# arpitbansal297/Cold-Diffusion-Models

Measured on NVIDIA H100. Metric: training-step images/sec (CelebA-128 deblur UNet, config 3), higher is better.
Workload: dtype tf32

## Files before the change

### cold_diffusion_models_b200/csrc/wgrad_tc.cu

```cuda
#include "tc_common.cuh"

namespace {

constexpr int kMmaWarps = 8;
constexpr int kThreads = 32 * (kMmaWarps + 1);
constexpr int kMaxTaps = 8;
constexpr int kMaxGroups = 4;
constexpr int kMaxAccCols = 256;

struct WgParams {
  int B, Hg, Wg;
  int CW, R, KR;
  int chunks_x, chunks_y, total_chunks, chunks_per_split, splits;
  int Cout, Cin;
  int tiles_co, tiles_ci;
  int ngroups;
  int ntaps[kMaxGroups];
  int nloads[kMaxGroups];
  int tap_index[kMaxGroups][kMaxTaps];
  int tap_load[kMaxGroups][kMaxTaps];
  int tap_shift[kMaxGroups][kMaxTaps];
  int load_dy[kMaxGroups][kMaxTaps], load_dx[kMaxGroups][kMaxTaps];
  int halo;
  int sy, sx;
  int oys, oxs, oy0, ox0;
  int per_batch, chunks_per_img, splits_per_img;
  long long dw_batch_stride;
  float* dw;
  float* db;
  int wm_nbox[kMaxGroups], ci_tile;
  int wm_box[kMaxGroups][kMaxTaps][2], wm_shift[kMaxGroups][kMaxTaps][2], wm_tap[kMaxGroups][kMaxTaps][2];
};

__device__ __forceinline__ float lds_sw(const uint8_t* base, int row, int c) {
  return cd_round_tf32(*reinterpret_cast<const float*>(base + row * 128 + ((((c >> 2) ^ row) & 7) << 4) + (c & 3) * 4));
}
__device__ __forceinline__ void mma_tf32_16x8x8(float (&d)[4], const float (&a)[4], const float (&b)[2]) {
  asm volatile("mma.sync.aligned.m16n8k8.row.col.f32.tf32.tf32.f32 {%0, %1, %2, %3}, {%4, %5, %6, %7}, {%8, %9}, {%0, %1, %2, %3};"
               : "+f"(d[0]), "+f"(d[1]), "+f"(d[2]), "+f"(d[3])
               : "r"(__float_as_uint(a[0])), "r"(__float_as_uint(a[1])), "r"(__float_as_uint(a[2])), "r"(__float_as_uint(a[3])),
                 "r"(__float_as_uint(b[0])), "r"(__float_as_uint(b[1])));
}
__device__ __forceinline__ void red_add_v2(float* addr, float a, float b) {
  asm volatile("red.global.add.v2.f32 [%0], {%1, %2};" :: "l"(addr), "f"(a), "f"(b) : "memory");
}

template <int BN, int NT, bool BIAS>
__global__ void __launch_bounds__(kThreads, 1)
wgrad_tc_kernel(const __grid_constant__ CUtensorMap mapDY, const __grid_constant__ CUtensorMap mapX,
                const WgParams p, int stages, int a_bytes, int b_bytes, int b_tx_bytes) {
  constexpr int NCH = BN / 32;
  constexpr int NJ = BN / 16;
  static_assert(NT * BN <= kMaxAccCols, "accumulators of one CTA");
  extern __shared__ uint8_t smem_raw[];
  const uint32_t raw_addr = smem_u32(smem_raw);
  uint8_t* smem = smem_raw + ((1024u - (raw_addr & 1023u)) & 1023u);
  const int g = blockIdx.z;
  const int nl = p.nloads[g];
  const int stage_bytes = a_bytes + nl * b_bytes;
  uint64_t* bars = reinterpret_cast<uint64_t*>(smem + stages * stage_bytes);
  uint64_t* full_bar = bars;
  uint64_t* empty_bar = bars + stages;
  const int warp = threadIdx.x >> 5, lane = threadIdx.x & 31;

  if (threadIdx.x == 0) {
    for (int i = 0; i < stages; ++i) { mbar_init(&full_bar[i], 1); mbar_init(&empty_bar[i], kMmaWarps); }
    asm volatile("fence.mbarrier_init.release.cluster;" ::: "memory");
  }
  __syncthreads();

  const int tile = blockIdx.x;
  const int co0 = (tile % p.tiles_co) * 128, ci0 = (tile / p.tiles_co) * BN;
  const int split = blockIdx.y;
  int c_beg = split * p.chunks_per_split;
  int c_end = c_beg + p.chunks_per_split; if (c_end > p.total_chunks) c_end = p.total_chunks;
  long long dw_off = 0;
  if (p.per_batch) {
    const int n = split / p.splits_per_img, sp = split % p.splits_per_img;
    c_beg = n * p.chunks_per_img + sp * p.chunks_per_split;
    c_end = c_beg + p.chunks_per_split;
    if (c_end > (n + 1) * p.chunks_per_img) c_end = (n + 1) * p.chunks_per_img;
    dw_off = n * p.dw_batch_stride;
  }
  const int nchunks = c_end > c_beg ? c_end - c_beg : 0;

  if (warp == kMmaWarps) {
    for (int it = 0; it < nchunks; ++it) {
      const int c = c_beg + it;
      const int cx = c % p.chunks_x;
      const int cy = (c / p.chunks_x) % p.chunks_y;
      const int n = c / (p.chunks_x * p.chunks_y);
      const int gx0 = cx * p.CW, gy0 = cy * p.R;
      const uint32_t stage = it % stages, ph = (it / stages) & 1u;
      mbar_wait(&empty_bar[stage], ph ^ 1u);
      if (elect_one()) {
        mbar_expect_tx(&full_bar[stage], a_bytes + nl * b_tx_bytes);
        const uint32_t sa = smem_u32(smem + stage * stage_bytes);
#pragma unroll
        for (int ch = 0; ch < 4; ++ch)
          tma_load_4d(sa + ch * (a_bytes / 4), &mapDY, &full_bar[stage], co0 + ch * 32, gx0 * p.oxs + p.ox0, gy0 * p.oys + p.oy0, n);
        for (int l = 0; l < nl; ++l) {
          const uint32_t sb = sa + a_bytes + l * b_bytes;
          const int xin = gx0 * p.sx + p.load_dx[g][l], yin = gy0 * p.sy + p.load_dy[g][l];
          for (int ch = 0; ch < NCH; ++ch)
            tma_load_4d(sb + ch * (b_bytes / NCH), &mapX, &full_bar[stage], ci0 + ch * 32, xin, yin, n);
        }
      }
      __syncwarp();
    }
    return;
  }

  const int wm = warp & 3, wn = warp >> 2;
  const int gq = lane >> 2, tq = lane & 3;
  const bool bias_cta = BIAS && p.db != nullptr && (tile / p.tiles_co) == 0 && g == 0 && wn == 0;
  int tap_load[NT], tap_shift[NT];
#pragma unroll
  for (int t = 0; t < NT; ++t) { tap_load[t] = p.tap_load[g][t]; tap_shift[t] = p.tap_shift[g][t]; }
  float acc[NT][2][NJ][4];
#pragma unroll
  for (int t = 0; t < NT; ++t)
#pragma unroll
    for (int i = 0; i < 2; ++i)
#pragma unroll
      for (int j = 0; j < NJ; ++j)
#pragma unroll
        for (int e = 0; e < 4; ++e) acc[t][i][j][e] = 0.f;
  float bsum[2][2] = {{0.f, 0.f}, {0.f, 0.f}};
  const int ksteps = p.KR / 8, cw_shift = __ffs(p.CW) - 1, rowlen = p.CW + p.halo;
  for (int it = 0; it < nchunks; ++it) {
    const uint32_t stage = it % stages, ph = (it / stages) & 1u;
    mbar_wait(&full_bar[stage], ph);
    const uint8_t* sA = smem + stage * stage_bytes + wm * (a_bytes / 4);
    const uint8_t* sB = smem + stage * stage_bytes + a_bytes;
#pragma unroll 1
    for (int ks = 0; ks < ksteps; ++ks) {
      const int k0 = ks * 8 + tq, k1 = k0 + 4;
      float a[2][4];
#pragma unroll
      for (int i = 0; i < 2; ++i) {
        a[i][0] = lds_sw(sA, k0, i * 16 + gq);
        a[i][1] = lds_sw(sA, k0, i * 16 + gq + 8);
        a[i][2] = lds_sw(sA, k1, i * 16 + gq);
        a[i][3] = lds_sw(sA, k1, i * 16 + gq + 8);
        if (bias_cta) { bsum[i][0] += a[i][0] + a[i][2]; bsum[i][1] += a[i][1] + a[i][3]; }
      }
      const int r0 = (k0 >> cw_shift) * rowlen + (k0 & (p.CW - 1)), r1 = (k1 >> cw_shift) * rowlen + (k1 & (p.CW - 1));
#pragma unroll
      for (int t = 0; t < NT; ++t) {
        const uint8_t* sBt = sB + tap_load[t] * b_bytes;
#pragma unroll
        for (int j = 0; j < NJ; ++j) {
          const int cl = wn * (BN / 2) + j * 8 + gq;
          const uint8_t* sBc = sBt + (cl >> 5) * (b_bytes / NCH);
          const float b[2] = {lds_sw(sBc, r0 + tap_shift[t], cl & 31), lds_sw(sBc, r1 + tap_shift[t], cl & 31)};
          mma_tf32_16x8x8(acc[t][0][j], a[0], b);
          mma_tf32_16x8x8(acc[t][1][j], a[1], b);
        }
      }
    }
    __syncwarp();
    if (lane == 0) mbar_arrive(&empty_bar[stage]);
  }
  if (nchunks == 0) return;
#pragma unroll
  for (int t = 0; t < NT; ++t) {
    if (t >= p.ntaps[g]) break;
#pragma unroll
    for (int i = 0; i < 2; ++i) {
#pragma unroll
      for (int h = 0; h < 2; ++h) {
        const int co = co0 + wm * 32 + i * 16 + gq + h * 8;
        if (co >= p.Cout) continue;
        float* wrow = p.dw + dw_off + (static_cast<long long>(p.tap_index[g][t]) * p.Cout + co) * p.Cin;
#pragma unroll
        for (int j = 0; j < NJ; ++j) {
          const int ci = ci0 + wn * (BN / 2) + j * 8 + tq * 2;
          if (ci < p.Cin) red_add_v2(wrow + ci, acc[t][i][j][2 * h], acc[t][i][j][2 * h + 1]);
        }
      }
    }
  }
  if (BIAS && bias_cta) {
#pragma unroll
    for (int i = 0; i < 2; ++i)
#pragma unroll
      for (int h = 0; h < 2; ++h) {
        float v = bsum[i][h];
        v += __shfl_xor_sync(0xffffffffu, v, 1);
        v += __shfl_xor_sync(0xffffffffu, v, 2);
        const int co = co0 + wm * 32 + i * 16 + gq + h * 8;
        if (tq == 0 && co < p.Cout) atomicAdd(p.db + co, v);
      }
  }
}

constexpr int kWmThreads = 512;
constexpr int kWmKR = 64;
constexpr int kWmRegsLow = 40, kWmRegsHigh = 216;

template <int CW, bool HALO> struct WmGeom {
  static constexpr int R = kWmKR / CW, RL = HALO ? CW + 8 : CW;
  static constexpr int kXBox = RL * (R + (HALO ? 2 : 0)) * 128;
  static_assert(kXBox % 1024 == 0, "X boxes keep 1024-byte alignment");
};
template <int BN> struct WmTiles {
  static constexpr int kRawBox = kWmKR * 128;
  static constexpr int kRawBytes = (BN / 32) * kRawBox;
  static constexpr int kBBytes = BN * kWmKR * 4;
};
constexpr int wm_slots_1x1(int BN) { return BN == 128 ? 3 : 4; }
template <int BN, int CW, bool HALO> struct WmStage {
  static constexpr int kXBytes = (HALO ? 2 : 2 * wm_slots_1x1(BN)) * WmGeom<CW, HALO>::kXBox;
  static constexpr int kBytes = WmTiles<BN>::kRawBytes + WmTiles<BN>::kBBytes + kXBytes;
  static_assert((224 * 1024) / kBytes >= 2, "two stages of the wgmma weight-gradient kernel fit shared memory");
};

template <int BN, int NTW, int CW, bool HALO>
__device__ __forceinline__ void wm_consume(const WgParams& p, const uint8_t* smem, int stages, int stage_bytes,
                                           uint64_t* afull, uint64_t* aempty, uint64_t* bfull, uint64_t* bempty, int nchunks, int g,
                                           int tbeg, int co0, int ci0) {
  using G = WmGeom<CW, HALO>;
  using T = WmTiles<BN>;
  const int lane = threadIdx.x & 31, w = (threadIdx.x & 127) >> 5, gq = lane >> 2, tq = lane & 3;
  int off[NTW][2];
  const int c = 16 * (w & 1) + gq;
#pragma unroll
  for (int t = 0; t < NTW; ++t) {
#pragma unroll
    for (int h = 0; h < 2; ++h) {
      const int row = ((NTW <= 2 && p.Cin == 32) ? p.wm_shift[g][tbeg + t][w >> 1] : p.wm_shift[g][tbeg + t][0]) + 2 * tq + h;
      const int box = (NTW <= 2 && p.Cin == 32) ? 0 : (HALO ? 0 : 2 * (tbeg + t)) + (w >> 1);
      off[t][h] = box * G::kXBox + row * 128 + ((((c >> 2) ^ row) & 7) << 4) + (c & 3) * 4;
    }
  }
  float acc[NTW][BN / 2];
  uint32_t fr[2][NTW][4];
  auto load_frags = [&](uint32_t (&f)[NTW][4], const uint8_t* xs, int ks) {
    const int kofs = (((ks * 8) / CW) * G::RL + (ks * 8) % CW) * 128;
#pragma unroll
    for (int t = 0; t < NTW; ++t)
#pragma unroll
      for (int e = 0; e < 4; ++e)
        f[t][e] = __float_as_uint(cd_round_tf32(*reinterpret_cast<const float*>(xs + (off[t][e >> 1] ^ ((e & 1) * 32)) + kofs)));
  };
  if (nchunks == 0) return;
  mbar_wait(&afull[0], 0);
  load_frags(fr[0], smem + T::kRawBytes + T::kBBytes, 0);
  for (int it = 0; it < nchunks; ++it) {
    const uint32_t s = it % stages, ph = (it / stages) & 1u;
    mbar_wait(&bfull[s], ph);
    const uint8_t* xs = smem + s * stage_bytes + T::kRawBytes + T::kBBytes;
    const uint32_t bs = smem_u32(smem + s * stage_bytes + T::kRawBytes);
#pragma unroll
    for (int ks = 0; ks < kWmKR / 8; ++ks) {
      wgmma_fence();
      const uint64_t db = make_kmajor_sw128_desc(bs + (ks >> 2) * (BN * 128)) + uint64_t((ks & 3) * 2);
#pragma unroll
      for (int t = 0; t < NTW; ++t) wgmma_tf32_rs<BN>(acc[t], fr[ks & 1][t], db, (it | ks) != 0 ? 1u : 0u);
      wgmma_commit();
      if (ks + 1 < kWmKR / 8) {
        load_frags(fr[(ks + 1) & 1], xs, ks + 1);
      } else if (it + 1 < nchunks) {
        const uint32_t s1 = (it + 1) % stages, ph1 = ((it + 1) / stages) & 1u;
        mbar_wait(&afull[s1], ph1);
        load_frags(fr[0], smem + s1 * stage_bytes + T::kRawBytes + T::kBBytes, 0);
      }
      wgmma_wait<0>();
    }
    __syncwarp();
    if (lane == 0) { mbar_arrive(&aempty[s]); mbar_arrive(&bempty[s]); }
  }
  asm volatile("" ::: "memory");
  const long long dw_off = p.per_batch ? (blockIdx.y / p.splits_per_img) * p.dw_batch_stride : 0;
#pragma unroll
  for (int t = 0; t < NTW; ++t) {
    const int tap = p.wm_tap[g][tbeg + t][w >> 1];
    if (tap < 0) continue;
    float* wt = p.dw + dw_off + static_cast<long long>(tap) * p.Cout * p.Cin + ci0 + 32 * p.wm_box[g][tbeg + t][w >> 1] +
                16 * (w & 1) + gq;
#pragma unroll
    for (int j = 0; j < BN / 8; ++j)
#pragma unroll
      for (int e = 0; e < 4; ++e) {
        const int co = co0 + 8 * j + 2 * tq + (e & 1);
        if (co < p.Cout) atomicAdd(wt + static_cast<long long>(co) * p.Cin + (e >> 1) * 8, acc[t][4 * j + e]);
      }
  }
}

template <int BN, int NT, int CW, bool HALO>
__global__ void __launch_bounds__(kWmThreads, 1)
wgrad_wgmma_kernel(const __grid_constant__ CUtensorMap mapDY, const __grid_constant__ CUtensorMap mapX, const __grid_constant__ WgParams p,
                   int stages) {
  using G = WmGeom<CW, HALO>;
  using T = WmTiles<BN>;
  constexpr int kStage = WmStage<BN, CW, HALO>::kBytes;
  extern __shared__ uint8_t smem_raw[];
  const uint32_t raw_addr = smem_u32(smem_raw);
  uint8_t* smem = smem_raw + ((1024u - (raw_addr & 1023u)) & 1023u);
  uint64_t* bars = reinterpret_cast<uint64_t*>(smem + stages * kStage);
  uint64_t* afull = bars;
  uint64_t* aempty = bars + stages;
  uint64_t* rfull = bars + 2 * stages;
  uint64_t* rempty = bars + 3 * stages;
  uint64_t* bfull = bars + 4 * stages;
  uint64_t* bempty = bars + 5 * stages;
  const int warp = threadIdx.x >> 5, lane = threadIdx.x & 31, wg = threadIdx.x >> 7;
  const int g = blockIdx.z, nt = p.ntaps[g];
  const int ncons = nt > 1 ? 2 : 1;
  if (threadIdx.x == 0) {
    for (int i = 0; i < stages; ++i) {
      mbar_init(&afull[i], 1); mbar_init(&aempty[i], 4 * ncons);
      mbar_init(&rfull[i], 1); mbar_init(&rempty[i], 4);
      mbar_init(&bfull[i], 4); mbar_init(&bempty[i], 4 * ncons);
    }
    asm volatile("fence.mbarrier_init.release.cluster;" ::: "memory");
  }
  __syncthreads();

  const int tile = blockIdx.x;
  const int co0 = (tile % p.tiles_co) * BN, ci0 = (tile / p.tiles_co) * p.ci_tile;
  int c_beg = blockIdx.y * p.chunks_per_split;
  int c_end = c_beg + p.chunks_per_split; if (c_end > p.total_chunks) c_end = p.total_chunks;
  if (p.per_batch) {
    const int n = blockIdx.y / p.splits_per_img, sp = blockIdx.y % p.splits_per_img;
    c_beg = n * p.chunks_per_img + sp * p.chunks_per_split;
    c_end = c_beg + p.chunks_per_split;
    if (c_end > (n + 1) * p.chunks_per_img) c_end = (n + 1) * p.chunks_per_img;
  }
  const int nchunks = c_end > c_beg ? c_end - c_beg : 0;

  if (wg == 0) {
    asm volatile("setmaxnreg.dec.sync.aligned.u32 %0;" :: "n"(kWmRegsLow));
    if (warp != 0) return;
    for (int it = 0; it < nchunks; ++it) {
      const int ch = c_beg + it;
      const int gx0 = (ch % p.chunks_x) * CW, gy0 = ((ch / p.chunks_x) % p.chunks_y) * G::R, n = ch / (p.chunks_x * p.chunks_y);
      const uint32_t s = it % stages, ph = (it / stages) & 1u;
      const uint32_t sx = smem_u32(smem + s * kStage);
      mbar_wait(&rempty[s], ph ^ 1u);
      if (elect_one()) {
        mbar_expect_tx(&rfull[s], T::kRawBytes);
#pragma unroll
        for (int b = 0; b < BN / 32; ++b)
          tma_load_4d(sx + b * T::kRawBox, &mapDY, &rfull[s], co0 + 32 * b, gx0, gy0, n);
      }
      __syncwarp();
      mbar_wait(&aempty[s], ph ^ 1u);
      if (elect_one()) {
        const int nb = p.wm_nbox[g], h = HALO ? 1 : 0;
        mbar_expect_tx(&afull[s], nb * G::kXBox);
        for (int b = 0; b < nb; ++b)
          tma_load_4d(sx + T::kRawBytes + T::kBBytes + b * G::kXBox, &mapX, &afull[s], ci0 + 32 * b, gx0 - h, gy0 - h, n);
      }
      __syncwarp();
    }
    return;
  }
  if (wg == 1) {
    asm volatile("setmaxnreg.dec.sync.aligned.u32 %0;" :: "n"(kWmRegsLow));
    const int w4 = warp & 3;
    for (int it = 0; it < nchunks; ++it) {
      const uint32_t s = it % stages, ph = (it / stages) & 1u;
      mbar_wait(&rfull[s], ph);
      mbar_wait(&bempty[s], ph ^ 1u);
      const uint8_t* raw = smem + s * kStage;
      uint8_t* bt = smem + s * kStage + T::kRawBytes;
#pragma unroll 4
      for (int u = w4; u < (BN / 32) * (kWmKR / 4); u += 4) {
        const int b = u % (BN / 32), kq = u / (BN / 32);
        const int co = 32 * b + lane;
        const uint8_t* src = raw + b * T::kRawBox + (lane & 3) * 4;
        float v[4];
#pragma unroll
        for (int j = 0; j < 4; ++j) {
          const int px = 8 * (kq >> 1) + (kq & 1) + 2 * j;
          v[j] = cd_round_tf32(*reinterpret_cast<const float*>(src + px * 128 + ((((lane >> 2) ^ px) & 7) << 4)));
        }
        *reinterpret_cast<float4*>(bt + (kq >> 3) * (BN * 128) + co * 128 + (((kq ^ co) & 7) << 4)) = make_float4(v[0], v[1], v[2], v[3]);
      }
      asm volatile("fence.proxy.async.shared::cta;" ::: "memory");
      __syncwarp();
      if (lane == 0) { mbar_arrive(&rempty[s]); mbar_arrive(&bfull[s]); }
    }
    return;
  }
  const int half = (nt + 1) / 2;
  const int tbeg = (wg - 2) * half;
  const int ntw = wg == 2 ? half : nt - half;
  if (ntw <= 0) return;
  asm volatile("setmaxnreg.inc.sync.aligned.u32 %0;" :: "n"(kWmRegsHigh));
#define WM_CONSUME(n) wm_consume<BN, n, CW, HALO>(p, smem, stages, kStage, afull, aempty, bfull, bempty, nchunks, g, tbeg, co0, ci0)
  if constexpr (NT == 4 && HALO) {
    if (ntw == 4) WM_CONSUME(4);
    else if (ntw == 3) WM_CONSUME(3);
    else if (ntw == 2) WM_CONSUME(2);
    else WM_CONSUME(1);
  } else {
    if (ntw == 2) WM_CONSUME(2);
    else WM_CONSUME(1);
  }
#undef WM_CONSUME
}

int g_wg_mode = 1;

constexpr int kMaxSmem = 224 * 1024 + 1024 + 256;

template <int BN, int NT>
int launch_wg(bool bias, dim3 grid, size_t smem, cudaStream_t st, const CUtensorMap& mapDY, const CUtensorMap& mapX,
              const WgParams& p, int stages, int a_bytes, int b_bytes, int b_tx) {
  constexpr auto with_bias = wgrad_tc_kernel<BN, NT, true>, without = wgrad_tc_kernel<BN, NT, false>;
  CD_CUDA(bias ? smem_limit_once<with_bias>(kMaxSmem) : smem_limit_once<without>(kMaxSmem));
  auto kern = bias ? with_bias : without;
  kern<<<grid, kThreads, smem, st>>>(mapDY, mapX, p, stages, a_bytes, b_bytes, b_tx);
  CD_LAUNCH_CHECK();
  return 0;
}

}

extern "C" int cd_wgrad_tc_set_mode(int mode) { g_wg_mode = mode; return 0; }

static int g_wg_bias_fusion = 0;
extern "C" int cd_wgrad_tc_set_bias_fusion(int enable) { g_wg_bias_fusion = enable; return 0; }

static int g_split_policy = 3;
static int g_split_over_clk = 12000;
extern "C" int cd_wgrad_tc_set_split(int policy, int over_clk) { g_split_policy = policy; if (over_clk > 0) g_split_over_clk = over_clk; return 0; }

static int choose_splits(int tg, int total_chunks, int max_splits, double chunk_clk) {
  const int sms = cd_num_sms();
  if (max_splits < 1) max_splits = 1;
  int s;
  if (g_split_policy == 0) s = cd_cdiv(2 * sms, tg);
  else if (g_split_policy == 1) s = sms / tg;
  else if (g_split_policy == 2) s = 2 * sms / tg;
  else {
    double best = 1e30; s = 1;
    for (int c = 1; c <= max_splits && c * tg <= 4 * sms + tg; ++c) {
      const int cps = cd_cdiv(total_chunks, c);
      const int real = cd_cdiv(total_chunks, cps);
      const double cost = double(cd_cdiv(static_cast<long long>(tg) * real, sms)) * (cps * chunk_clk + g_split_over_clk);
      if (cost < best) { best = cost; s = c; }
    }
  }
  if (s > max_splits) s = max_splits;
  if (s < 1) s = 1;
  return s;
}

template <int BN, int NT, int CW, bool HALO>
static int launch_wm(dim3 grid, cudaStream_t st, const CUtensorMap& mapDY, const CUtensorMap& mapX, const WgParams& p) {
  constexpr int kStage = WmStage<BN, CW, HALO>::kBytes;
  int stages = (224 * 1024) / kStage; if (stages > 5) stages = 5;
  const size_t smem = size_t(stages) * kStage + 1024 + 256;
  constexpr auto kern = wgrad_wgmma_kernel<BN, NT, CW, HALO>;
  CD_CUDA(smem_limit_once<kern>(kMaxSmem));
  kern<<<grid, kWmThreads, smem, st>>>(mapDY, mapX, p, stages);
  CD_LAUNCH_CHECK();
  return 0;
}

struct WmClass { int ey, ex, n, tap[16], sy[16], sx[16]; };

static int wm_plan(const CdConvDesc* d, const WmClass& k, int BN, int CW, WgParams& p, bool& halo) {
  const int Cin = d->s[0].C, NT = BN == 128 ? 2 : 4;
  halo = !(k.n == 1 && k.sy[0] == 0 && k.sx[0] == 0);
  p.tiles_co = d->Cout / BN;
  int sb[16][2], ss[16][2], st[16][2], ns = 0, nbox = 2;
  auto shift = [&](int i) { return halo ? (k.sy[i] + 1) * (CW + 8) + k.sx[i] + 1 : 0; };
  if (Cin == 32) {
    if (halo && BN != 128) return 1;
    nbox = 1;
    for (int i = 0; i < k.n; i += 2, ++ns)
      for (int h = 0; h < 2; ++h) {
        const bool on = i + h < k.n;
        sb[ns][h] = 0; ss[ns][h] = on ? shift(i + h) : 0; st[ns][h] = on ? k.tap[i + h] : -1;
      }
  } else if (!halo) {
    ns = wm_slots_1x1(BN);
    while ((Cin / 64) % ns != 0) --ns;
    nbox = 2 * ns;
    for (int t = 0; t < ns; ++t)
      for (int h = 0; h < 2; ++h) { sb[t][h] = 2 * t + h; ss[t][h] = 0; st[t][h] = k.tap[0]; }
  } else {
    for (int i = 0; i < k.n; ++i, ++ns)
      for (int h = 0; h < 2; ++h) { sb[ns][h] = h; ss[ns][h] = shift(i); st[ns][h] = k.tap[i]; }
  }
  p.ci_tile = Cin == 32 ? 32 : 32 * nbox;
  p.tiles_ci = Cin == 32 ? 1 : Cin / p.ci_tile;
  p.ngroups = cd_cdiv(ns, 2 * NT);
  if (p.ngroups > kMaxGroups) return 1;
  for (int g = 0; g < p.ngroups; ++g) {
    const int s0 = g * 2 * NT, n = ns - s0 < 2 * NT ? ns - s0 : 2 * NT;
    p.ntaps[g] = n;
    p.wm_nbox[g] = nbox;
    for (int t = 0; t < n; ++t)
      for (int h = 0; h < 2; ++h) { p.wm_box[g][t][h] = sb[s0 + t][h]; p.wm_shift[g][t][h] = ss[s0 + t][h]; p.wm_tap[g][t][h] = st[s0 + t][h]; }
  }
  return 0;
}

static int wgrad_wgmma(const CdConvDesc* d, const float* dout, int dout_ld, float* dw, cudaStream_t st) {
  const CdConvSrc& c = d->s[0];
  if ((c.C % 64 != 0 && c.C != 32) || d->Cout % 64 != 0 || c.ntaps < 1) return 1;
  const bool dense_out = d->oys == 1 && d->oxs == 1 && d->oy0 == 0 && d->ox0 == 0 && d->Ho == d->Hg && d->Wo == d->Wg;
  const bool parity_out = d->oys == 2 && d->oxs == 2 && (d->oy0 & ~1) == 0 && (d->ox0 & ~1) == 0 && d->Ho == 2 * d->Hg &&
                          d->Wo == 2 * d->Wg;
  const bool s1 = d->sy == 1 && d->sx == 1 && c.H == d->Hg && c.W == d->Wg && (dense_out || parity_out);
  const bool s2 = d->sy == 2 && d->sx == 2 && c.H == 2 * d->Hg && c.W == 2 * d->Wg && dense_out;
  if (!s1 && !s2) return 1;
  const int CW = d->Wg >= 16 ? 16 : 8, R = kWmKR / CW;
  if (d->Hg < R) return 1;
  const int BN = d->Cout % 128 == 0 ? 128 : 64;
  WmClass cls[4];
  int ncls = 0;
  for (int e = 0; e < (s2 ? 4 : 1); ++e) {
    WmClass& k = cls[ncls];
    k.ey = e >> 1; k.ex = e & 1; k.n = 0;
    for (int t = 0; t < c.ntaps; ++t) {
      if (s2 && ((c.dy[t] & 1) != k.ey || (c.dx[t] & 1) != k.ex)) continue;
      const int sy = s2 ? (c.dy[t] - k.ey) / 2 : c.dy[t], sx = s2 ? (c.dx[t] - k.ex) / 2 : c.dx[t];
      if (sy < -1 || sy > 1 || sx < -1 || sx > 1) return 1;
      k.tap[k.n] = t; k.sy[k.n] = sy; k.sx[k.n] = sx; ++k.n;
    }
    if (k.n > 0) ++ncls;
  }
  WgParams ps[4];
  bool halo[4];
  for (int i = 0; i < ncls; ++i) {
    ps[i] = WgParams{};
    if (wm_plan(d, cls[i], BN, CW, ps[i], halo[i])) return 1;
  }
  CUtensorMap mapDY;
  if (!encode_nhwc(&mapDY, CU_TENSOR_MAP_DATA_TYPE_FLOAT32, dout, dout_ld, d->Cout, d->Wo, d->Ho, d->B, d->oxs, d->oys, d->ox0, d->oy0,
                   CW, R, 1, 1, 1, "wgmma dY"))
    return -1;
  for (int i = 0; i < ncls; ++i) {
    WgParams& p = ps[i];
    p.B = d->B; p.Hg = d->Hg; p.Wg = d->Wg; p.Cout = d->Cout; p.Cin = c.C;
    p.dw = dw;
    p.CW = CW; p.R = R; p.KR = kWmKR;
    p.chunks_x = d->Wg / CW; p.chunks_y = d->Hg / R;
    p.total_chunks = d->B * p.chunks_x * p.chunks_y;
    const int tiles = p.tiles_co * p.tiles_ci;
    const double chunk_clk = double(p.ntaps[0]) * (kWmKR / 8) * (BN / 2);
    if (c.w_per_batch) {
      p.per_batch = 1;
      p.chunks_per_img = p.chunks_x * p.chunks_y;
      const int spi = choose_splits(tiles * p.ngroups * d->B, p.chunks_per_img, p.chunks_per_img, chunk_clk);
      p.chunks_per_split = cd_cdiv(p.chunks_per_img, spi);
      p.splits_per_img = cd_cdiv(p.chunks_per_img, p.chunks_per_split);
      p.splits = p.splits_per_img * d->B;
      p.dw_batch_stride = static_cast<long long>(c.ntaps) * d->Cout * c.C;
    } else {
      const int splits = choose_splits(tiles * p.ngroups, p.total_chunks, cd_cdiv(p.total_chunks, 8), chunk_clk);
      p.chunks_per_split = cd_cdiv(p.total_chunks, splits);
      p.splits = cd_cdiv(p.total_chunks, p.chunks_per_split);
    }
    CUtensorMap mapX;
    const int bw = halo[i] ? CW + 8 : CW, bh = halo[i] ? R + 2 : R;
    if (!encode_nhwc(&mapX, CU_TENSOR_MAP_DATA_TYPE_FLOAT32, c.src, c.ld, c.C, c.W, c.H, d->B, d->sx, d->sy, cls[i].ex, cls[i].ey, bw, bh,
                     1, 1, 1, "wgmma X"))
      return -1;
    const dim3 grid(tiles, p.splits, p.ngroups);
#define WM_LAUNCH(bn, nt, cw) (halo[i] ? launch_wm<bn, nt, cw, true>(grid, st, mapDY, mapX, p) \
                                       : launch_wm<bn, nt, cw, false>(grid, st, mapDY, mapX, p))
    int rc;
    if (BN == 128) rc = CW == 16 ? WM_LAUNCH(128, 2, 16) : WM_LAUNCH(128, 2, 8);
    else rc = CW == 16 ? WM_LAUNCH(64, 4, 16) : WM_LAUNCH(64, 4, 8);
#undef WM_LAUNCH
    if (rc) return rc;
  }
  return 0;
}

int cd_conv_wgrad_tc(const CdConvDesc* d, const float* dout, int dout_ld, float* dw, float* db, int* bias_done, cudaStream_t st) {
  if (bias_done) *bias_done = 0;
  const CdConvSrc& c = d->s[0];
  if (c.C % 32 != 0 || d->Cout % 32 != 0 || c.ld % 4 != 0 || dout_ld % 4 != 0) return 1;
  if (!is_pow2(d->Wg) || d->Wg < 8 || !is_pow2(d->Hg)) return 1;
  if ((reinterpret_cast<uintptr_t>(c.src) & 15) || (reinterpret_cast<uintptr_t>(dout) & 15) || (reinterpret_cast<uintptr_t>(dw) & 15)) return 1;
  if (g_wg_mode != 0 && g_wg_mode != 8 && !(g_wg_bias_fusion && db != nullptr)) {
    const int r = wgrad_wgmma(d, dout, dout_ld, dw, st);
    if (r <= 0) return r;
  }

  WgParams p{};
  p.B = d->B; p.Hg = d->Hg; p.Wg = d->Wg; p.Cout = d->Cout; p.Cin = c.C;
  p.sy = d->sy; p.sx = d->sx; p.oys = d->oys; p.oxs = d->oxs; p.oy0 = d->oy0; p.ox0 = d->ox0;
  p.dw = dw;
  int BN = c.C >= 128 ? 128 : 64;
  const bool is3x3 = (c.ntaps == 9 && d->sy == 1 && d->sx == 1);
  bool shape3 = is3x3;
  if (is3x3) for (int t = 0; t < 9; ++t) if (c.dy[t] != t / 3 - 1 || c.dx[t] != t % 3 - 1) shape3 = false;
  const bool halo = shape3 && g_wg_mode != 0;
  p.halo = halo ? 2 : 0;
  if (halo) {
    p.ngroups = 3;
    for (int gk = 0; gk < 3; ++gk) {
      p.ntaps[gk] = 3; p.nloads[gk] = 1; p.load_dy[gk][0] = gk - 1; p.load_dx[gk][0] = -1;
      for (int k = 0; k < 3; ++k) { p.tap_index[gk][k] = gk * 3 + k; p.tap_load[gk][k] = 0; p.tap_shift[gk][k] = k; }
    }
  } else {
    const int per = c.ntaps <= 4 ? c.ntaps : (c.ntaps == 9 ? 3 : 4);
    if (c.ntaps % per != 0 || c.ntaps / per > kMaxGroups) return 1;
    p.ngroups = c.ntaps / per;
    for (int gk = 0; gk < p.ngroups; ++gk) {
      p.ntaps[gk] = per; p.nloads[gk] = per;
      for (int k = 0; k < per; ++k) {
        const int t = gk * per + k;
        p.tap_index[gk][k] = t; p.tap_load[gk][k] = k; p.tap_shift[gk][k] = 0;
        p.load_dy[gk][k] = c.dy[t]; p.load_dx[gk][k] = c.dx[t];
      }
    }
  }
  const int max_taps = p.ntaps[0], max_loads = p.nloads[0];
  if (max_taps * BN > kMaxAccCols) BN = 64;
  if (max_taps * BN > kMaxAccCols) return 1;
  int KR = (max_loads <= 1) ? 64 : 32;
  if (static_cast<long long>(d->Hg) * d->Wg < KR) KR = d->Hg * d->Wg;
  if (KR < 8) return 1;
  p.CW = d->Wg < KR ? d->Wg : KR;
  p.R = KR / p.CW;
  p.KR = KR;
  if (p.CW * d->sx > 256 || p.CW * d->oxs > 256) return 1;
  p.chunks_x = d->Wg / p.CW; p.chunks_y = d->Hg / p.R;
  p.total_chunks = d->B * p.chunks_x * p.chunks_y;
  p.tiles_co = cd_cdiv(d->Cout, 128); p.tiles_ci = cd_cdiv(c.C, BN);
  const int tiles = p.tiles_co * p.tiles_ci;
  const double chunk_clk = double(max_taps) * (KR / 8) * (BN == 128 ? 256.0 : 128.0);
  int splits;
  if (c.w_per_batch) {
    const int cpi = p.chunks_x * p.chunks_y;
    const int spi0 = choose_splits(tiles * p.ngroups * d->B, cpi, cpi, chunk_clk);
    splits = spi0 * d->B;
  } else {
    splits = choose_splits(tiles * p.ngroups, p.total_chunks, cd_cdiv(p.total_chunks, 8), chunk_clk);
  }
  p.chunks_per_split = cd_cdiv(p.total_chunks, splits);
  p.splits = cd_cdiv(p.total_chunks, p.chunks_per_split);
  if (c.w_per_batch) {
    p.per_batch = 1;
    p.chunks_per_img = p.chunks_x * p.chunks_y;
    int spi = cd_cdiv(splits, d->B); if (spi < 1) spi = 1; if (spi > p.chunks_per_img) spi = p.chunks_per_img;
    p.chunks_per_split = cd_cdiv(p.chunks_per_img, spi);
    p.splits_per_img = cd_cdiv(p.chunks_per_img, p.chunks_per_split);
    p.splits = p.splits_per_img * d->B;
    p.dw_batch_stride = static_cast<long long>(c.ntaps) * d->Cout * c.C;
  }
  const int a_bytes = 4 * KR * 128;
  const int b_rows = p.R * (p.CW + p.halo);
  const int b_rows_pad = (b_rows + 7) / 8 * 8;
  const int b_bytes = (BN / 32) * b_rows_pad * 128;
  const int b_tx = (BN / 32) * b_rows * 128;
  const int stage_bytes = a_bytes + max_loads * b_bytes;
  int stages = (224 * 1024) / stage_bytes; if (stages > 6) stages = 6;
  if (stages < 2) return 1;
  const bool fuse_bias = g_wg_bias_fusion && db != nullptr && !c.w_per_batch && d->oys == 1 && d->oxs == 1;
  p.db = fuse_bias ? db : nullptr;
  const size_t smem = size_t(stages) * stage_bytes + 1024 + 256;

  CUtensorMap mapDY, mapX;
  const CUtensorMapDataType dt = CU_TENSOR_MAP_DATA_TYPE_FLOAT32;
  if (!encode_nhwc(&mapDY, dt, dout, dout_ld, d->Cout, d->Wo, d->Ho, d->B, 1, 1, 0, 0, p.CW * d->oxs, p.R * d->oys, 1, d->oxs, d->oys,
                   "dY") ||
      !encode_nhwc(&mapX, dt, c.src, c.ld, c.C, c.W, c.H, d->B, 1, 1, 0, 0, (p.CW + p.halo) * d->sx, p.R * d->sy, 1, d->sx, d->sy, "X"))
    return -1;
  dim3 grid(tiles, p.splits, p.ngroups);
  int rc;
  if (BN == 128) rc = max_taps == 1 ? launch_wg<128, 1>(fuse_bias, grid, smem, st, mapDY, mapX, p, stages, a_bytes, b_bytes, b_tx)
                                    : launch_wg<128, 2>(fuse_bias, grid, smem, st, mapDY, mapX, p, stages, a_bytes, b_bytes, b_tx);
  else if (max_taps == 1) rc = launch_wg<64, 1>(fuse_bias, grid, smem, st, mapDY, mapX, p, stages, a_bytes, b_bytes, b_tx);
  else if (max_taps == 2) rc = launch_wg<64, 2>(fuse_bias, grid, smem, st, mapDY, mapX, p, stages, a_bytes, b_bytes, b_tx);
  else if (max_taps == 3) rc = launch_wg<64, 3>(fuse_bias, grid, smem, st, mapDY, mapX, p, stages, a_bytes, b_bytes, b_tx);
  else rc = launch_wg<64, 4>(fuse_bias, grid, smem, st, mapDY, mapX, p, stages, a_bytes, b_bytes, b_tx);
  if (rc == 0 && fuse_bias && bias_done) *bias_done = 1;
  return rc;
}
```

Before: 703.5.

## Make wgmma weight-gradient kernel persistent with balanced tap groups and overlapped waits

Turns the wgmma weight-gradient kernel into a persistent kernel. A grid capped at the SM count walks a flattened list of (tile, group, split) items, and the mbarrier phase counters carry across items so the TMA pipeline keeps running between work items. Taps are now spread evenly across groups, and the BN=64 path drops from up to 4 taps per warpgroup to 3. The consumer waits with wgmma_wait<1> so the next fragment loads overlap the running MMA. It also adds plan-recording and skip-item debug hooks, and consumer warpgroups with no taps now drain barriers instead of exiting. The aim is to cut launch tail and load imbalance, at the cost of more complex barrier bookkeeping and a possible loss of parallelism when there are few items.

```diff
diff --git a/cold_diffusion_models_b200/csrc/wgrad_tc.cu b/cold_diffusion_models_b200/csrc/wgrad_tc.cu
--- a/cold_diffusion_models_b200/csrc/wgrad_tc.cu
+++ b/cold_diffusion_models_b200/csrc/wgrad_tc.cu
@@ -30,6 +30,7 @@
   float* db;
   int wm_nbox[kMaxGroups], ci_tile;
   int wm_box[kMaxGroups][kMaxTaps][2], wm_shift[kMaxGroups][kMaxTaps][2], wm_tap[kMaxGroups][kMaxTaps][2];
+  int skip_item;
 };
 
 __device__ __forceinline__ float lds_sw(const uint8_t* base, int row, int c) {
@@ -216,10 +217,32 @@
   static_assert((224 * 1024) / kBytes >= 2, "two stages of the wgmma weight-gradient kernel fit shared memory");
 };
 
+struct WmItem { int co0, ci0, g, c_beg, nchunks; long long dw_off; };
+template <int BN>
+__device__ __forceinline__ WmItem wm_item(const WgParams& p, int item) {
+  const int tiles = p.tiles_co * p.tiles_ci;
+  const int tile = item % tiles, g = (item / tiles) % p.ngroups, split = item / (tiles * p.ngroups);
+  WmItem w;
+  w.co0 = (tile % p.tiles_co) * BN; w.ci0 = (tile / p.tiles_co) * p.ci_tile; w.g = g;
+  int c_end;
+  if (p.per_batch) {
+    const int n = split / p.splits_per_img, sp = split % p.splits_per_img;
+    w.c_beg = n * p.chunks_per_img + sp * p.chunks_per_split;
+    c_end = min(w.c_beg + p.chunks_per_split, (n + 1) * p.chunks_per_img);
+    w.dw_off = n * p.dw_batch_stride;
+  } else {
+    w.c_beg = split * p.chunks_per_split;
+    c_end = min(w.c_beg + p.chunks_per_split, p.total_chunks);
+    w.dw_off = 0;
+  }
+  w.nchunks = c_end > w.c_beg && item != p.skip_item ? c_end - w.c_beg : 0;
+  return w;
+}
+
 template <int BN, int NTW, int CW, bool HALO>
 __device__ __forceinline__ void wm_consume(const WgParams& p, const uint8_t* smem, int stages, int stage_bytes,
-                                           uint64_t* afull, uint64_t* aempty, uint64_t* bfull, uint64_t* bempty, int nchunks, int g,
-                                           int tbeg, int co0, int ci0) {
+                                           uint64_t* afull, uint64_t* aempty, uint64_t* bfull, uint64_t* bempty, uint32_t it0,
+                                           int nchunks, int g, int tbeg, int co0, int ci0, long long dw_off) {
   using G = WmGeom<CW, HALO>;
   using T = WmTiles<BN>;
   const int lane = threadIdx.x & 31, w = (threadIdx.x & 127) >> 5, gq = lane >> 2, tq = lane & 3;
@@ -235,6 +258,10 @@
     }
   }
   float acc[NTW][BN / 2];
+#pragma unroll
+  for (int t = 0; t < NTW; ++t)
+#pragma unroll
+    for (int j = 0; j < BN / 2; ++j) acc[t][j] = 0.f;
   uint32_t fr[2][NTW][4];
   auto load_frags = [&](uint32_t (&f)[NTW][4], const uint8_t* xs, int ks) {
     const int kofs = (((ks * 8) / CW) * G::RL + (ks * 8) % CW) * 128;
@@ -245,10 +272,13 @@
         f[t][e] = __float_as_uint(cd_round_tf32(*reinterpret_cast<const float*>(xs + (off[t][e >> 1] ^ ((e & 1) * 32)) + kofs)));
   };
   if (nchunks == 0) return;
-  mbar_wait(&afull[0], 0);
-  load_frags(fr[0], smem + T::kRawBytes + T::kBBytes, 0);
+  {
+    const uint32_t s0 = it0 % stages;
+    mbar_wait(&afull[s0], (it0 / stages) & 1u);
+    load_frags(fr[0], smem + s0 * stage_bytes + T::kRawBytes + T::kBBytes, 0);
+  }
   for (int it = 0; it < nchunks; ++it) {
-    const uint32_t s = it % stages, ph = (it / stages) & 1u;
+    const uint32_t s = (it0 + it) % stages, ph = ((it0 + it) / stages) & 1u;
     mbar_wait(&bfull[s], ph);
     const uint8_t* xs = smem + s * stage_bytes + T::kRawBytes + T::kBBytes;
     const uint32_t bs = smem_u32(smem + s * stage_bytes + T::kRawBytes);
@@ -259,20 +289,22 @@
 #pragma unroll
       for (int t = 0; t < NTW; ++t) wgmma_tf32_rs<BN>(acc[t], fr[ks & 1][t], db, (it | ks) != 0 ? 1u : 0u);
       wgmma_commit();
+      wgmma_wait<1>();
       if (ks + 1 < kWmKR / 8) {
         load_frags(fr[(ks + 1) & 1], xs, ks + 1);
-      } else if (it + 1 < nchunks) {
-        const uint32_t s1 = (it + 1) % stages, ph1 = ((it + 1) / stages) & 1u;
-        mbar_wait(&afull[s1], ph1);
-        load_frags(fr[0], smem + s1 * stage_bytes + T::kRawBytes + T::kBBytes, 0);
-      }
-      wgmma_wait<0>();
+      } else {
+        if (it + 1 < nchunks) {
+          const uint32_t s1 = (it0 + it + 1) % stages, ph1 = ((it0 + it + 1) / stages) & 1u;
+          mbar_wait(&afull[s1], ph1);
+          load_frags(fr[0], smem + s1 * stage_bytes + T::kRawBytes + T::kBBytes, 0);
+        }
+        wgmma_wait<0>();
+      }
     }
     __syncwarp();
     if (lane == 0) { mbar_arrive(&aempty[s]); mbar_arrive(&bempty[s]); }
   }
   asm volatile("" ::: "memory");
-  const long long dw_off = p.per_batch ? (blockIdx.y / p.splits_per_img) * p.dw_batch_stride : 0;
 #pragma unroll
   for (int t = 0; t < NTW; ++t) {
     const int tap = p.wm_tap[g][tbeg + t][w >> 1];
@@ -307,61 +339,54 @@
   uint64_t* bfull = bars + 4 * stages;
   uint64_t* bempty = bars + 5 * stages;
   const int warp = threadIdx.x >> 5, lane = threadIdx.x & 31, wg = threadIdx.x >> 7;
-  const int g = blockIdx.z, nt = p.ntaps[g];
-  const int ncons = nt > 1 ? 2 : 1;
   if (threadIdx.x == 0) {
     for (int i = 0; i < stages; ++i) {
-      mbar_init(&afull[i], 1); mbar_init(&aempty[i], 4 * ncons);
+      mbar_init(&afull[i], 1); mbar_init(&aempty[i], 8);
       mbar_init(&rfull[i], 1); mbar_init(&rempty[i], 4);
-      mbar_init(&bfull[i], 4); mbar_init(&bempty[i], 4 * ncons);
+      mbar_init(&bfull[i], 4); mbar_init(&bempty[i], 8);
     }
     asm volatile("fence.mbarrier_init.release.cluster;" ::: "memory");
   }
   __syncthreads();
-
-  const int tile = blockIdx.x;
-  const int co0 = (tile % p.tiles_co) * BN, ci0 = (tile / p.tiles_co) * p.ci_tile;
-  int c_beg = blockIdx.y * p.chunks_per_split;
-  int c_end = c_beg + p.chunks_per_split; if (c_end > p.total_chunks) c_end = p.total_chunks;
-  if (p.per_batch) {
-    const int n = blockIdx.y / p.splits_per_img, sp = blockIdx.y % p.splits_per_img;
-    c_beg = n * p.chunks_per_img + sp * p.chunks_per_split;
-    c_end = c_beg + p.chunks_per_split;
-    if (c_end > (n + 1) * p.chunks_per_img) c_end = (n + 1) * p.chunks_per_img;
-  }
-  const int nchunks = c_end > c_beg ? c_end - c_beg : 0;
+  const int nitems = p.tiles_co * p.tiles_ci * p.ngroups * p.splits;
 
   if (wg == 0) {
     asm volatile("setmaxnreg.dec.sync.aligned.u32 %0;" :: "n"(kWmRegsLow));
     if (warp != 0) return;
-    for (int it = 0; it < nchunks; ++it) {
-      const int ch = c_beg + it;
-      const int gx0 = (ch % p.chunks_x) * CW, gy0 = ((ch / p.chunks_x) % p.chunks_y) * G::R, n = ch / (p.chunks_x * p.chunks_y);
-      const uint32_t s = it % stages, ph = (it / stages) & 1u;
-      const uint32_t sx = smem_u32(smem + s * kStage);
-      mbar_wait(&rempty[s], ph ^ 1u);
-      if (elect_one()) {
-        mbar_expect_tx(&rfull[s], T::kRawBytes);
-#pragma unroll
-        for (int b = 0; b < BN / 32; ++b)
-          tma_load_4d(sx + b * T::kRawBox, &mapDY, &rfull[s], co0 + 32 * b, gx0, gy0, n);
-      }
-      __syncwarp();
-      mbar_wait(&aempty[s], ph ^ 1u);
-      if (elect_one()) {
-        const int nb = p.wm_nbox[g], h = HALO ? 1 : 0;
-        mbar_expect_tx(&afull[s], nb * G::kXBox);
-        for (int b = 0; b < nb; ++b)
-          tma_load_4d(sx + T::kRawBytes + T::kBBytes + b * G::kXBox, &mapX, &afull[s], ci0 + 32 * b, gx0 - h, gy0 - h, n);
-      }
-      __syncwarp();
+    uint32_t it = 0;
+    for (int item = blockIdx.x; item < nitems; item += gridDim.x) {
+      const WmItem w = wm_item<BN>(p, item);
+      for (int c = 0; c < w.nchunks; ++c, ++it) {
+        const int ch = w.c_beg + c;
+        const int gx0 = (ch % p.chunks_x) * CW, gy0 = ((ch / p.chunks_x) % p.chunks_y) * G::R, n = ch / (p.chunks_x * p.chunks_y);
+        const uint32_t s = it % stages, ph = (it / stages) & 1u;
+        const uint32_t sx = smem_u32(smem + s * kStage);
+        mbar_wait(&rempty[s], ph ^ 1u);
+        if (elect_one()) {
+          mbar_expect_tx(&rfull[s], T::kRawBytes);
+#pragma unroll
+          for (int b = 0; b < BN / 32; ++b)
+            tma_load_4d(sx + b * T::kRawBox, &mapDY, &rfull[s], w.co0 + 32 * b, gx0, gy0, n);
+        }
+        __syncwarp();
+        mbar_wait(&aempty[s], ph ^ 1u);
+        if (elect_one()) {
+          const int nb = p.wm_nbox[w.g], h = HALO ? 1 : 0;
+          mbar_expect_tx(&afull[s], nb * G::kXBox);
+          for (int b = 0; b < nb; ++b)
+            tma_load_4d(sx + T::kRawBytes + T::kBBytes + b * G::kXBox, &mapX, &afull[s], w.ci0 + 32 * b, gx0 - h, gy0 - h, n);
+        }
+        __syncwarp();
+      }
     }
     return;
   }
   if (wg == 1) {
     asm volatile("setmaxnreg.dec.sync.aligned.u32 %0;" :: "n"(kWmRegsLow));
     const int w4 = warp & 3;
-    for (int it = 0; it < nchunks; ++it) {
+    uint32_t nchunks = 0;
+    for (int item = blockIdx.x; item < nitems; item += gridDim.x) nchunks += wm_item<BN>(p, item).nchunks;
+    for (uint32_t it = 0; it < nchunks; ++it) {
       const uint32_t s = it % stages, ph = (it / stages) & 1u;
       mbar_wait(&rfull[s], ph);
       mbar_wait(&bempty[s], ph ^ 1u);
@@ -386,22 +411,34 @@
     }
     return;
   }
-  const int half = (nt + 1) / 2;
-  const int tbeg = (wg - 2) * half;
-  const int ntw = wg == 2 ? half : nt - half;
-  if (ntw <= 0) return;
   asm volatile("setmaxnreg.inc.sync.aligned.u32 %0;" :: "n"(kWmRegsHigh));
-#define WM_CONSUME(n) wm_consume<BN, n, CW, HALO>(p, smem, stages, kStage, afull, aempty, bfull, bempty, nchunks, g, tbeg, co0, ci0)
-  if constexpr (NT == 4 && HALO) {
-    if (ntw == 4) WM_CONSUME(4);
-    else if (ntw == 3) WM_CONSUME(3);
-    else if (ntw == 2) WM_CONSUME(2);
-    else WM_CONSUME(1);
-  } else {
-    if (ntw == 2) WM_CONSUME(2);
-    else WM_CONSUME(1);
-  }
+  uint32_t it0 = 0;
+  for (int item = blockIdx.x; item < nitems; item += gridDim.x) {
+    const WmItem w = wm_item<BN>(p, item);
+    const int nt = p.ntaps[w.g], half = (nt + 1) / 2;
+    const int tbeg = (wg - 2) * half;
+    const int ntw = wg == 2 ? half : nt - half;
+#define WM_CONSUME(n) wm_consume<BN, n, CW, HALO>(p, smem, stages, kStage, afull, aempty, bfull, bempty, it0, w.nchunks, w.g, tbeg, \
+                                                  w.co0, w.ci0, w.dw_off)
+    if (ntw <= 0) {
+      for (int it = 0; it < w.nchunks; ++it) {
+        const uint32_t s = (it0 + it) % stages, ph = ((it0 + it) / stages) & 1u;
+        mbar_wait(&afull[s], ph);
+        mbar_wait(&bfull[s], ph);
+        __syncwarp();
+        if (lane == 0) { mbar_arrive(&aempty[s]); mbar_arrive(&bempty[s]); }
+      }
+    } else if constexpr (NT == 3 && HALO) {
+      if (ntw == 3) WM_CONSUME(3);
+      else if (ntw == 2) WM_CONSUME(2);
+      else WM_CONSUME(1);
+    } else {
+      if (ntw == 2) WM_CONSUME(2);
+      else WM_CONSUME(1);
+    }
 #undef WM_CONSUME
+    it0 += w.nchunks;
+  }
 }
 
 int g_wg_mode = 1;
@@ -427,8 +464,13 @@
 extern "C" int cd_wgrad_tc_set_bias_fusion(int enable) { g_wg_bias_fusion = enable; return 0; }
 
 static int g_split_policy = 3;
-static int g_split_over_clk = 12000;
-extern "C" int cd_wgrad_tc_set_split(int policy, int over_clk) { g_split_policy = policy; if (over_clk > 0) g_split_over_clk = over_clk; return 0; }
+constexpr int kItemClk = 12000;
+static int g_split_over_clk = kItemClk;
+extern "C" int cd_wgrad_tc_set_split(int policy, int over_clk) {
+  g_split_policy = policy;
+  g_split_over_clk = over_clk > 0 ? over_clk : kItemClk;
+  return 0;
+}
 
 static int choose_splits(int tg, int total_chunks, int max_splits, double chunk_clk) {
   const int sms = cd_num_sms();
@@ -452,13 +494,13 @@
 }
 
 template <int BN, int NT, int CW, bool HALO>
-static int launch_wm(dim3 grid, cudaStream_t st, const CUtensorMap& mapDY, const CUtensorMap& mapX, const WgParams& p) {
+static int launch_wm(int items, cudaStream_t st, const CUtensorMap& mapDY, const CUtensorMap& mapX, const WgParams& p) {
   constexpr int kStage = WmStage<BN, CW, HALO>::kBytes;
   int stages = (224 * 1024) / kStage; if (stages > 5) stages = 5;
   const size_t smem = size_t(stages) * kStage + 1024 + 256;
   constexpr auto kern = wgrad_wgmma_kernel<BN, NT, CW, HALO>;
   CD_CUDA(smem_limit_once<kern>(kMaxSmem));
-  kern<<<grid, kWmThreads, smem, st>>>(mapDY, mapX, p, stages);
+  kern<<<items < cd_num_sms() ? items : cd_num_sms(), kWmThreads, smem, st>>>(mapDY, mapX, p, stages);
   CD_LAUNCH_CHECK();
   return 0;
 }
@@ -466,7 +508,7 @@
 struct WmClass { int ey, ex, n, tap[16], sy[16], sx[16]; };
 
 static int wm_plan(const CdConvDesc* d, const WmClass& k, int BN, int CW, WgParams& p, bool& halo) {
-  const int Cin = d->s[0].C, NT = BN == 128 ? 2 : 4;
+  const int Cin = d->s[0].C, NT = BN == 128 ? 2 : 3;
   halo = !(k.n == 1 && k.sy[0] == 0 && k.sx[0] == 0);
   p.tiles_co = d->Cout / BN;
   int sb[16][2], ss[16][2], st[16][2], ns = 0, nbox = 2;
@@ -493,17 +535,28 @@
   p.tiles_ci = Cin == 32 ? 1 : Cin / p.ci_tile;
   p.ngroups = cd_cdiv(ns, 2 * NT);
   if (p.ngroups > kMaxGroups) return 1;
-  for (int g = 0; g < p.ngroups; ++g) {
-    const int s0 = g * 2 * NT, n = ns - s0 < 2 * NT ? ns - s0 : 2 * NT;
+  for (int g = 0, s0 = 0; g < p.ngroups; ++g) {
+    const int n = ns / p.ngroups + (g < ns % p.ngroups ? 1 : 0);
     p.ntaps[g] = n;
     p.wm_nbox[g] = nbox;
     for (int t = 0; t < n; ++t)
       for (int h = 0; h < 2; ++h) { p.wm_box[g][t][h] = sb[s0 + t][h]; p.wm_shift[g][t][h] = ss[s0 + t][h]; p.wm_tap[g][t][h] = st[s0 + t][h]; }
+    s0 += n;
   }
   return 0;
 }
 
+static int g_wm_plan[1 + 8 * 4];
+extern "C" int cd_wgrad_tc_last_plan(int* out, int n) {
+  for (int i = 0; i < n && i < 1 + 8 * 4; ++i) out[i] = g_wm_plan[i];
+  return 0;
+}
+
+static int g_wm_skip_item = -1;
+extern "C" int cd_wgrad_tc_set_skip_item(int item) { g_wm_skip_item = item; return 0; }
+
 static int wgrad_wgmma(const CdConvDesc* d, const float* dout, int dout_ld, float* dw, cudaStream_t st) {
+  g_wm_plan[0] = 0;
   const CdConvSrc& c = d->s[0];
   if ((c.C % 64 != 0 && c.C != 32) || d->Cout % 64 != 0 || c.ntaps < 1) return 1;
   const bool dense_out = d->oys == 1 && d->oxs == 1 && d->oy0 == 0 && d->ox0 == 0 && d->Ho == d->Hg && d->Wo == d->Wg;
@@ -540,6 +593,7 @@
     return -1;
   for (int i = 0; i < ncls; ++i) {
     WgParams& p = ps[i];
+    p.skip_item = g_wm_skip_item;
     p.B = d->B; p.Hg = d->Hg; p.Wg = d->Wg; p.Cout = d->Cout; p.Cin = c.C;
     p.dw = dw;
     p.CW = CW; p.R = R; p.KR = kWmKR;
@@ -565,12 +619,17 @@
     if (!encode_nhwc(&mapX, CU_TENSOR_MAP_DATA_TYPE_FLOAT32, c.src, c.ld, c.C, c.W, c.H, d->B, d->sx, d->sy, cls[i].ex, cls[i].ey, bw, bh,
                      1, 1, 1, "wgmma X"))
       return -1;
-    const dim3 grid(tiles, p.splits, p.ngroups);
-#define WM_LAUNCH(bn, nt, cw) (halo[i] ? launch_wm<bn, nt, cw, true>(grid, st, mapDY, mapX, p) \
-                                       : launch_wm<bn, nt, cw, false>(grid, st, mapDY, mapX, p))
+    const int items = tiles * p.ngroups * p.splits;
+    int* rec = g_wm_plan + 1 + 8 * i;
+    rec[0] = items < cd_num_sms() ? items : cd_num_sms(); rec[1] = tiles; rec[2] = p.splits; rec[3] = p.chunks_per_split;
+    rec[4] = p.ngroups;
+    for (int k = 0; k < 3; ++k) rec[5 + k] = k < p.ngroups ? p.ntaps[k] : 0;
+    g_wm_plan[0] = i + 1;
+#define WM_LAUNCH(bn, nt, cw) (halo[i] ? launch_wm<bn, nt, cw, true>(items, st, mapDY, mapX, p) \
+                                       : launch_wm<bn, nt, cw, false>(items, st, mapDY, mapX, p))
     int rc;
     if (BN == 128) rc = CW == 16 ? WM_LAUNCH(128, 2, 16) : WM_LAUNCH(128, 2, 8);
-    else rc = CW == 16 ? WM_LAUNCH(64, 4, 16) : WM_LAUNCH(64, 4, 8);
+    else rc = CW == 16 ? WM_LAUNCH(64, 3, 16) : WM_LAUNCH(64, 3, 8);
 #undef WM_LAUNCH
     if (rc) return rc;
   }
```

New measurement: 714.3 (median of 6 runs). +1.5%, better.
